# QuantumLab-ZY/HamGNN

Hardware: AMD Instinct MI355X
Metric: edges/sec (equivariant MP forward) (higher is better)
Workload: dtype f32; 1 GPU; sio2_10k: 10002 atoms, 822350 directed edges, irreps set-A (D=877), sh lmax 5, 3 layers, nao_max 19, no SOC, backbone+head forward; parallelism=single GPU

## Files before the change

hamgnn_amd/csrc/tp_is.hip:

```cpp
#include "tp_stage.h"

#ifdef HG_PROF
__device__ unsigned long long hg_prof_is_acc[16];
struct ProfIs { unsigned long long t[12]; unsigned long long last; };
#define IS_PROF_ARG , ProfIs& prof
#define IS_PROF_PASS , prof
#define IS_T(k)                                                      \
    do {                                                             \
        const unsigned long long t_ = __builtin_readcyclecounter();  \
        prof.t[k] += t_ - prof.last;                                 \
        prof.last = t_;                                              \
    } while (0)
#else
#define IS_PROF_ARG
#define IS_PROF_PASS
#define IS_T(k)
#endif
#define IS_MB_CASE(Q) case Q: asm("v_mul_f32_dpp %0, %1, %2 row_newbcast:" #Q " row_mask:0xf bank_mask:0xf" : "=v"(o) : "v"(v), "v"(x)); break;
__device__ __forceinline__ float is_mul_bcast(float v, float x, int q) {
    float o;
    switch (q) {
        IS_MB_CASE(0) IS_MB_CASE(1) IS_MB_CASE(2) IS_MB_CASE(3) IS_MB_CASE(4) IS_MB_CASE(5) IS_MB_CASE(6) IS_MB_CASE(7)
        IS_MB_CASE(8) IS_MB_CASE(9) IS_MB_CASE(10) IS_MB_CASE(11) IS_MB_CASE(12) IS_MB_CASE(13) IS_MB_CASE(14)
        default: asm("v_mul_f32_dpp %0, %1, %2 row_newbcast:15 row_mask:0xf bank_mask:0xf" : "=v"(o) : "v"(v), "v"(x)); break;
    }
    return o;
}
#undef IS_MB_CASE

template <int MM, int RTM, bool SPLIT, bool ODD>
__device__ __forceinline__ void item_is(const IsArgs& A, const float* __restrict__ Wb, const int* __restrict__ it,
                                        float* __restrict__ lds, int64_t erow, int lane, const IsHidden& hbr, int hbr_cls IS_PROF_ARG) {
    constexpr int NCR = 2 * MM + 1;
    constexpr int NC = ODD ? 2 * MM : NCR;
#define IS_COL(c) ((ODD && (c) >= MM) ? (c) + 1 : (c))
#define IS_NK2_OK(rt, r) ((rt) + 1 < RTM || 4 * (rt) + (r) < nk2)
    constexpr int CW = NC > 7 ? (NC + 1) / 2 : NC;
    const int typ = it[0], so0 = it[1], so1 = it[2], in_mulp = it[4], li = it[5], neg = it[7];
    const int ksteps = it[8], mlp = it[10], x4 = it[17], nk2 = it[18];
    const int rto = it[22];
    const int g = lane >> 4, el = lane & 15;
    const int* __restrict__ rtab = reinterpret_cast<const int*>(lds + A.rowtab_off) + it[23];
    float* __restrict__ tbase = lds + (SPLIT ? A.tile_shift : 0) + (el - MM * 16);
    const float* __restrict__ stage = lds + A.stage_off;
    IS_T(0);

    const int nsrc = so1 >= 0 ? 2 : 1;
    const int ngrp = (ksteps + 3) >> 2;
    const f32x4* __restrict__ aw = reinterpret_cast<const f32x4*>(Wb + it[11]) + lane;
    f32x4 av_n[RTM];
    constexpr int NPAIR = RTM * NCR, NJ = (NPAIR + 15) / 16;
    f32x4 cfv[NJ];
    if (typ == 0) {
        const f32x4* __restrict__ cfp = reinterpret_cast<const f32x4*>(Wb + it[13] + NPAIR * 16) + lane;
#pragma unroll
        for (int j = 0; j < NJ; ++j) cfv[j] = cfp[j * 64];
    }
    f32x4 S[RTM];
    if (typ == 0) {
#pragma unroll
        for (int rt = 0; rt < RTM; ++rt) S[rt] = (f32x4){0.f, 0.f, 0.f, 0.f};
        const float* __restrict__ hrow = (mlp ? A.h2[1] : A.h2[0]) + erow * A.hidden + 4 * g;
        const f32x4* __restrict__ w3 = reinterpret_cast<const f32x4*>(Wb + it[12]) + lane;
        const int hgrp = A.hidden >> 4;
        if (mlp == hbr_cls) {
            const f32x4* __restrict__ w3s = w3 + 4 * RTM * 64;
            f32x4 wh[2][RTM], wl[2][RTM], S1[RTM];
#pragma unroll
            for (int t = 0; t < 2; ++t)
#pragma unroll
                for (int rt = 0; rt < RTM; ++rt) {
                    wh[t][rt] = w3s[((t * RTM + rt) * 2) * 64];
                    wl[t][rt] = w3s[((t * RTM + rt) * 2 + 1) * 64];
                }
#pragma unroll
            for (int rt = 0; rt < RTM; ++rt) S1[rt] = (f32x4){0.f, 0.f, 0.f, 0.f};
#ifndef K_S_NOBATCH
            asm volatile("s_waitcnt vmcnt(0)" ::: "memory");
            __builtin_amdgcn_sched_barrier(0);
#endif
#pragma unroll
            for (int t = 0; t < 2; ++t) {
#pragma unroll
                for (int rt = 0; rt < RTM; ++rt) S[rt] = __builtin_amdgcn_mfma_f32_16x16x32_f16(__builtin_bit_cast(f16x8, wh[t][rt]), hbr.hi[t], S[rt], 0, 0, 0);
#pragma unroll
                for (int rt = 0; rt < RTM; ++rt) S1[rt] = __builtin_amdgcn_mfma_f32_16x16x32_f16(__builtin_bit_cast(f16x8, wh[t][rt]), hbr.lo[t], S1[rt], 0, 0, 0);
#pragma unroll
                for (int rt = 0; rt < RTM; ++rt) S1[rt] = __builtin_amdgcn_mfma_f32_16x16x32_f16(__builtin_bit_cast(f16x8, wl[t][rt]), hbr.hi[t], S1[rt], 0, 0, 0);
            }
#ifndef K_S_NOBATCH
            __builtin_amdgcn_sched_barrier(0);
#endif
            const float c0 = A.s_scale, c1 = A.s_scale * (1.f / 2048.f);
#pragma unroll
            for (int rt = 0; rt < RTM; ++rt) S[rt] = S[rt] * c0 + S1[rt] * c1;
        } else
#pragma unroll 1
        for (int G0 = 0; G0 < hgrp; G0 += 4) {
            f32x4 hb[4], wv[4][RTM];
#pragma unroll
            for (int G = 0; G < 4; ++G)
                if (G0 + G < hgrp) {
                    hb[G] = *reinterpret_cast<const f32x4*>(hrow + 16 * (G0 + G));
#pragma unroll
                    for (int rt = 0; rt < RTM; ++rt) wv[G][rt] = w3[((G0 + G) * RTM + rt) * 64];
                }
#pragma unroll
            for (int G = 0; G < 4; ++G)
                if (G0 + G < hgrp) {
#pragma unroll
                    for (int q = 0; q < 4; ++q)
#pragma unroll
                        for (int rt = 0; rt < RTM; ++rt) S[rt] = __builtin_amdgcn_mfma_f32_16x16x4f32(wv[G][rt][q], hb[G][q], S[rt], 0, 0, 0);
                }
        }
    }

    IS_T(1);
#if defined(K_XDL_DUMMY) || defined(K_SMFMA_DUMMY)
#ifdef K_XD_ROLE
    if (typ == 0 && ((blockIdx.x >> 8) & 1)) {
#else
    if (typ == 0) {
#endif
        f32x4 dA[RTM], dB[RTM];
#pragma unroll
        for (int rt = 0; rt < RTM; ++rt) dA[rt] = dB[rt] = (f32x4){0.f, 0.f, 0.f, 0.f};
#ifdef K_XD_DRAIN
// ... 67 lines not shown
#endif
#if defined(K_XD_DRAIN) || defined(K_XD_NOPS)
        __builtin_amdgcn_sched_barrier(0);
        asm volatile("s_nop 15\n s_nop 15\n s_nop 15\n s_nop 15" ::: "memory");
#ifdef K_XD_LONG
#pragma unroll 1
        for (int w_ = 0; w_ < K_XD_LONG; ++w_) asm volatile("s_nop 15\n s_nop 15\n s_nop 15\n s_nop 15" ::: "memory");
#endif
        __builtin_amdgcn_sched_barrier(0);
#endif
#pragma unroll
        for (int rt = 0; rt < RTM; ++rt) asm volatile("" :: "v"(dA[rt]), "v"(dB[rt]));
#if defined(K_XD_DRAIN)
        __builtin_amdgcn_sched_barrier(0);
#endif
    }
#endif
    f32x4 mid[RTM][NC];
#pragma unroll
    for (int rt = 0; rt < RTM; ++rt)
#pragma unroll
        for (int c = 0; c < NC; ++c) mid[rt][c] = (f32x4){0.f, 0.f, 0.f, 0.f};
    const int P1 = in_mulp >> 2;
    const int cdir = neg ? -P1 : P1;
    const int c0p = (li - MM) * P1 + (neg ? (NCR - 1) * P1 : 0);
    const int ntot = nsrc * ngrp;
    const int src_jump = (so1 - so0) - ngrp * 256;
    if (NCR <= 3 && x4) {
        const float* __restrict__ pc[NC];
#pragma unroll
        for (int c = 0; c < NC; ++c) pc[c] = stage + so0 + (c0p + g + IS_COL(c) * cdir) * 64 + el * 4;
#pragma unroll
        for (int rt = 0; rt < RTM; ++rt) av_n[rt] = aw[rt * 64];
#pragma unroll 1
        for (int t = 0; t < ntot; ++t) {
            if (t == ngrp) {
#pragma unroll
                for (int c = 0; c < NC; ++c) pc[c] += src_jump;
            }
            f32x4 av[RTM], bv[NC];
#pragma unroll
            for (int rt = 0; rt < RTM; ++rt) av[rt] = av_n[rt];
            if (t + 1 < ntot) {
#pragma unroll
                for (int rt = 0; rt < RTM; ++rt) av_n[rt] = aw[((t + 1) * RTM + rt) * 64];
            }
#pragma unroll
            for (int c = 0; c < NC; ++c) {
                bv[c] = *reinterpret_cast<const f32x4*>(pc[c]);
                pc[c] += 256;
            }
#pragma unroll
            for (int q = 0; q < 4; ++q)
#pragma unroll
                for (int rt = 0; rt < RTM; ++rt)
#pragma unroll
                    for (int c = 0; c < NC; ++c)
                        mid[rt][c] = __builtin_amdgcn_mfma_f32_16x16x4f32(av[rt][q], bv[c][q], mid[rt][c], 0, 0, 0);
        }
    } else {
        const float* __restrict__ pc[NC];
#pragma unroll
        for (int c = 0; c < NC; ++c) pc[c] = stage + so0 + (c0p + IS_COL(c) * cdir) * 64 + el * 4 + g;
#pragma unroll
        for (int rt = 0; rt < RTM; ++rt) av_n[rt] = aw[rt * 64];
        int nq = ksteps;
#pragma unroll 1
        for (int t = 0; t < ntot; ++t) {
            if (t == ngrp) {
                nq = ksteps;
#pragma unroll
                for (int c = 0; c < NC; ++c) pc[c] += src_jump;
            }
            f32x4 av[RTM];
#pragma unroll
            for (int rt = 0; rt < RTM; ++rt) av[rt] = av_n[rt];
            if (t + 1 < ntot) {
#pragma unroll
                for (int rt = 0; rt < RTM; ++rt) av_n[rt] = aw[((t + 1) * RTM + rt) * 64];
            }
#pragma unroll
            for (int q = 0; q < 4; ++q) {
                if (q < nq) {
                    float b[NC];
#pragma unroll
                    for (int c = 0; c < NC; ++c) b[c] = pc[c][q * 64];
                    __builtin_amdgcn_sched_barrier(0);
#pragma unroll
                    for (int rt = 0; rt < RTM; ++rt)
#pragma unroll
                        for (int c = 0; c < NC; ++c)
                            mid[rt][c] = __builtin_amdgcn_mfma_f32_16x16x4f32(av[rt][q], b[c], mid[rt][c], 0, 0, 0);
                }
            }
            nq -= 4;
#pragma unroll
            for (int c = 0; c < NC; ++c) pc[c] += 256;
        }
    }

    IS_T(2);
    if (typ == 0) {
        const f32x4* __restrict__ a2 = reinterpret_cast<const f32x4*>(Wb + it[14]) + lane;
        const f32x4* __restrict__ cf = reinterpret_cast<const f32x4*>(Wb + it[13]) + g;
        f32x4 a2_n[RTM];
#pragma unroll
        for (int rt = 0; rt < RTM; ++rt) a2_n[rt] = a2[rt * 64];
#pragma unroll
        for (int rt = 0; rt < RTM; ++rt)
#pragma unroll
            for (int c = 0; c < NC; ++c) {
                const int p = rt * NCR + IS_COL(c);
                f32x4 t = mid[rt][c] * S[rt];
#pragma unroll
                for (int r = 0; r < 4; ++r) t[r] = is_mul_bcast(cfv[p >> 4][r], t[r], p & 15);
                mid[rt][c] = t;
            }

        if (CW == NC) {
            float* __restrict__ tnext[4];
            f32x4 acc_n[NC];
#pragma unroll
            for (int r = 0; r < 4; ++r) tnext[r] = tbase + rtab[4 * g + r];
#pragma unroll
            for (int c = 0; c < NC; ++c)
#pragma unroll
                for (int r = 0; r < 4; ++r) acc_n[c][r] = tnext[r][IS_COL(c) * 16];
#pragma unroll 1
            for (int rtp = 0; rtp < rto; ++rtp) {
                f32x4 av[RTM], acc[NC];
                float* __restrict__ trow[4];
#pragma unroll
                for (int rt = 0; rt < RTM; ++rt) av[rt] = a2_n[rt];
// ... 365 lines not shown
#pragma unroll
                        for (int r = 0; r < 4; ++r) tb[rowoff[rtp][r] + (c0 + c) * 16] = acc[c][r];
                    }
            }
        } else {
#pragma unroll 1
            for (int rtp = 0; rtp < RTO; ++rtp) {
                f32x4 avr[RTO], acc[CH];
                int ro[4];
#pragma unroll
                for (int rt = 0; rt < RTO; ++rt) avr[rt] = a2[(rtp * RTO + rt) * 64];
#pragma unroll
                for (int r = 0; r < 4; ++r) ro[r] = rtab[16 * rtp + 4 * g + r];
#pragma unroll
                for (int c = 0; c < CH; ++c) acc[c] = (f32x4){0.f, 0.f, 0.f, 0.f};
#pragma unroll
                for (int rt = 0; rt < RTO; ++rt)
#pragma unroll
                    for (int r = 0; r < 4; ++r)
#pragma unroll
                        for (int c = 0; c < CH; ++c) acc[c] = __builtin_amdgcn_mfma_f32_16x16x4f32(avr[rt][r], md[rt][c][r], acc[c], 0, 0, 0);
#pragma unroll
                for (int c = 0; c < CH; ++c)
                    if (c0 + c < nco) {
#pragma unroll
                        for (int r = 0; r < 4; ++r) tb[ro[r] + (c0 + c) * 16] = acc[c][r];
                    }
            }
        }
    }
}

#define IS_CASE(MMv, RTMv) \
    case (MMv * 8 + RTMv): item_is<MMv, RTMv, SPLIT, false>(A, g_W, it, lds, erow, lane, hbr, hbr_cls IS_PROF_PASS); break;
#define IS_CASE_ODD(MMv, RTMv) \
    case (64 + MMv * 8 + RTMv): item_is<MMv, RTMv, SPLIT, true>(A, g_W, it, lds, erow, lane, hbr, hbr_cls IS_PROF_PASS); break;

#define IS_PART_I32 16

template <bool SPLIT, bool LITE>
__global__ __launch_bounds__(LITE ? 64 * IS_NW_LITE : IS_NT, (LITE ? IS_NW_LITE : IS_NW) / 2) void tp_is_kernel(const IsArgs A0, const int* __restrict__ g_segs, const int* __restrict__ g_blocks,
                                                       const int* __restrict__ g_phases, const int* __restrict__ g_groups,
                                                       const int* __restrict__ g_items, const float* __restrict__ g_W,
                                                       const int* __restrict__ g_parts, const int* __restrict__ g_rowtab) {
    extern __shared__ __attribute__((aligned(16))) float lds[];
    constexpr int NW = LITE ? IS_NW_LITE : IS_NW, NT = 64 * NW;
    const int wave = threadIdx.x >> 6, lane = threadIdx.x & 63;
    const int g = lane >> 4;
    const int64_t e = (int64_t)blockIdx.x * 16 + (lane & 15);
    const bool valid = e < A0.rows;
    const int64_t eslot = valid ? e : A0.rows - 1;
    const int64_t erow = A0.eperm ? A0.eperm[eslot] : eslot;
    const int* __restrict__ PT = g_parts + (SPLIT ? blockIdx.y : 0) * IS_PART_I32;
    IsArgs Asplit;
    if constexpr (SPLIT) {
        Asplit = A0;
        Asplit.trash_off = PT[4];
        Asplit.stage_off = PT[5];
        Asplit.ctr_off = PT[6];
        Asplit.rowtab_off = PT[8];
        Asplit.rowtab_begin = PT[9];
        Asplit.rowtab_len = PT[10];
        Asplit.tile_shift = wave * PT[7];
    }
    const IsArgs& A = SPLIT ? Asplit : A0;
    const int seg0 = SPLIT ? PT[0] : 0, seg1 = SPLIT ? PT[0] + PT[1] : A0.nseg, ph0 = SPLIT ? PT[2] : 0, ph1 = SPLIT ? PT[2] + PT[3] : A0.nphase;
    const int copy_stride = SPLIT ? PT[7] : 0;
    float* __restrict__ stage = lds + A.stage_off;
    int* __restrict__ ctr = reinterpret_cast<int*>(lds + A.ctr_off);
// ... 43 lines not shown
                case 1: stage_block<1, NW>(A, B, stage, erow, wave, lane); break;
                case 2: stage_block<2, NW>(A, B, stage, erow, wave, lane); break;
                case 3: stage_block<3, NW>(A, B, stage, erow, wave, lane); break;
                case 4: stage_block<4, NW>(A, B, stage, erow, wave, lane); break;
                case 5: stage_block<5, NW>(A, B, stage, erow, wave, lane); break;
                case 6: stage_block<6, NW>(A, B, stage, erow, wave, lane); break;
                default: break;
            }
#ifdef HG_PROF
            if (!((A.rot_mask >> B[0]) & 1)) { IS_T(8); } else if (B[4] == 0) { IS_T(9); } else if (B[4] <= 3) { IS_T(10); } else { IS_T(11); }
#endif
        }
        asm volatile("s_waitcnt vmcnt(0)" ::: "memory");
        __syncthreads();
        IS_T(6);
        int gi_dealt = g0 + __builtin_amdgcn_readfirstlane(wave);
        while (true) {
            int gi = 0;
#if defined(IS_DYNAMIC_CLAIM)
            if (false) {
#elif defined(IS_DEAL_ALL)
            if (true) {
#else
            if (SPLIT && copy_stride) {
#endif
                gi = gi_dealt;
                gi_dealt += NW;
            } else {
                if (lane == 0) gi = atomicAdd(ctr, 1);
                gi = __builtin_amdgcn_readfirstlane(gi);
            }
            if (gi >= g1) break;
            const int ib = g_groups[2 * gi], ie = g_groups[2 * gi + 1];
            for (int ii = ib; ii < ie; ++ii) {
                const int* __restrict__ it = g_items + ii * 24;
                if (LITE) {
                    IS_T(0);
                    if (it[0] == 3) {
                        if (it[22] == 1) post_is<1>(A, g_W, it, lds, erow, lane);
                        else if (it[22] == 2) post_is<2>(A, g_W, it, lds, erow, lane);
                        else if (it[22] == 3) post_is<3>(A, g_W, it, lds, erow, lane);
                        else post_is<4>(A, g_W, it, lds, erow, lane);
                    }
                    else if (it[0] == 6) stream_lite(A, g_W, it, lds, lane);
                    else if (it[9] == 1) item_lite<1>(A, g_W, it, lds, lane);
                    else if (it[9] == 2) item_lite<2>(A, g_W, it, lds, lane);
                    else if (it[9] == 3) item_lite<3>(A, g_W, it, lds, lane);
                    else item_lite<4>(A, g_W, it, lds, lane);
                    if (it[0] == 3) { IS_T(3); } else { IS_T(2); }
                    continue;
                }
                switch (it[6] * 8 + it[9] + ((it[0] == 0 && it[7]) ? 64 : 0)) {
                    IS_CASE(0, 1) IS_CASE(0, 2) IS_CASE(0, 3) IS_CASE(0, 4)
                    IS_CASE(1, 1) IS_CASE(1, 2) IS_CASE(1, 3) IS_CASE(1, 4)
                    IS_CASE(2, 1) IS_CASE(2, 2) IS_CASE(2, 3)
                    IS_CASE(3, 1) IS_CASE(3, 2)
                    IS_CASE(4, 1) IS_CASE(4, 2)
                    IS_CASE(5, 1)
                    IS_CASE(6, 1)
                    IS_CASE_ODD(1, 1) IS_CASE_ODD(1, 2) IS_CASE_ODD(1, 3) IS_CASE_ODD(1, 4)
                    IS_CASE_ODD(2, 1) IS_CASE_ODD(2, 2) IS_CASE_ODD(2, 3)
                    IS_CASE_ODD(3, 1) IS_CASE_ODD(3, 2)
                    IS_CASE_ODD(4, 1) IS_CASE_ODD(4, 2)
                    IS_CASE_ODD(5, 1)
                    IS_CASE_ODD(6, 1)
                    default: break;
                }
            }
        }
    }

    if (SPLIT && copy_stride) {
        __syncthreads();
        for (int i = threadIdx.x; i < copy_stride; i += NT) {
            float acc = lds[i];
#pragma unroll
            for (int k = 1; k < NW; ++k) acc += lds[i + k * copy_stride];
            lds[i] = acc;
        }
    }
    IsScan scan;
    scan.last = true, scan.row = 0;
    if (!SPLIT && A0.run_id) scan = is_scan_setup(valid ? A0.run_id[e] : -1 - (int)(lane & 15), lane & 15);
    for (int sg = seg0; sg < seg1; ++sg) {
        const int* __restrict__ S8 = g_segs + sg * 8;
        const int lk = S8[0], mul_k = S8[1], out_off = S8[3], out_mulp = S8[4], tile_off = S8[5], woff = S8[6], flags = S8[7];
        if (sg == seg0 || (flags & SEG_NEWBATCH)) {
            __syncthreads();
            if (flags & SEG_NEWBATCH) {
                int lprev = -1;
                for (int s2 = sg; s2 < seg1; ++s2) {
                    const int* __restrict__ T8 = g_segs + s2 * 8;
                    if (s2 > sg && (T8[7] & SEG_NEWBATCH)) break;
                    const int l2 = T8[0];
                    if (!(T8[7] & SEG_UNROTATE) || l2 == lprev) continue;
                    lprev = l2;
                    const int nn = (2 * l2 + 1) * (2 * l2 + 1);
                    const float* __restrict__ D = A.wig + erow * A.nW + is_pick_wig_off(A, l2);
                    const int nj = (nn + 3) >> 2;
// ... 53 lines not shown

extern "C" int hg_tp_is(const float* const* src, const int64_t* src_stride, int nsrc, const float* h2_node, const float* h2_edge,
                        int hidden, const float* wig, int nW, const int32_t* wig_off, const float* weights, const int32_t* seg_table,
                        const int32_t* block_table, const int32_t* phase_table, const int32_t* group_table,
                        const int32_t* item_table, const int32_t* part_table, const int32_t* part_table_host, int nparts,
                        const int32_t* row_table, int lds_bytes,
                        const int64_t* const* src_idx, int rot_mask, const int64_t* edge_perm, const int32_t* run_id, float* out, int64_t out_stride,
                        int64_t rows, void* stream) {
    HgDeviceGuard dev_guard(stream);
    if (rows <= 0) return 0;
    if (nsrc < 1 || nsrc > 4) return hg_fail(-2, "hg_tp_is: nsrc must be 1..4");
    if (hidden & 15) return hg_fail(-2, "hg_tp_is: (padded) hidden width must be a multiple of 16");
    if (lds_bytes <= 0 || lds_bytes > 160 * 1024) return hg_fail(-2, "hg_tp_is: bad LDS size");
    if (!part_table || !part_table_host || nparts < 1 || nparts > 64) return hg_fail(-2, "hg_tp_is: 1..64 parts");
    IsArgs A;
    for (int i = 0; i < 4; ++i) {
        A.src[i] = i < nsrc ? src[i] : src[0];
        A.sstride[i] = i < nsrc ? src_stride[i] : src_stride[0];
    }
    A.h2[0] = h2_node;
    A.h2[1] = h2_edge;
    A.hidden = hidden;
    A.wig = wig;
    A.nW = nW;
    for (int i = 0; i < 8; ++i) A.wig_off[i] = wig_off ? wig_off[i] : 0;
    A.out = out;
    A.ostride = out_stride;
    A.rows = rows;
    A.tile_shift = 0;
    const int32_t* p0 = part_table_host;
    A.nseg = p0[1], A.nphase = p0[3], A.trash_off = p0[4], A.stage_off = p0[5], A.ctr_off = p0[6];
    A.rowtab_off = p0[8], A.rowtab_begin = p0[9], A.rowtab_len = p0[10];
    A.s_split = p0[12] == 1 && hidden == 64;
    A.s_scale = ldexpf(1.f, -(p0[13] + IS_SPLIT_H_EXP));
    if (!row_table) return hg_fail(-2, "hg_tp_is: no row table");
    for (int p = 0; p < nparts; ++p) {
        const int32_t* q = part_table_host + p * IS_PART_I32;
        if (q[6] < q[5] || q[5] < q[8] + q[10] || q[8] < q[4] || lds_bytes < 4 * (q[6] + 1) || (q[7] && (part_table_host[11] ? IS_NW_LITE : IS_NW) * q[7] > q[8]))
            return hg_fail(-2, "hg_tp_is: bad LDS layout");
    }
    for (int i = 0; i < 4; ++i) A.idx[i] = (src_idx && i < nsrc) ? src_idx[i] : nullptr;
    A.rot_mask = rot_mask;
    A.eperm = edge_perm;
    A.run_id = run_id;
    if (run_id && nparts != 1) return hg_fail(-2, "hg_tp_is: the fused scatter needs a single-part launch");
    if (rot_mask && !wig) return hg_fail(-2, "hg_tp_is: rotated sources need the Wigner rows");
    static unsigned char lds_attr_done[4][HG_MAX_DEVICES];
    if (int rc = hg_lds_attr_once(lds_attr_done[0], dev_guard.dev, (const void*)tp_is_kernel<false, false>, 160 * 1024)) return rc;
    if (int rc = hg_lds_attr_once(lds_attr_done[1], dev_guard.dev, (const void*)tp_is_kernel<true, false>, 160 * 1024)) return rc;
    if (int rc = hg_lds_attr_once(lds_attr_done[2], dev_guard.dev, (const void*)tp_is_kernel<false, true>, 160 * 1024)) return rc;
    if (int rc = hg_lds_attr_once(lds_attr_done[3], dev_guard.dev, (const void*)tp_is_kernel<true, true>, 160 * 1024)) return rc;
    const unsigned grid = (unsigned)((rows + 15) / 16);
    const bool lite = p0[11] != 0;
#define IS_LAUNCH(SPLITv, LITEv, GRID) \
    hipLaunchKernelGGL((tp_is_kernel<SPLITv, LITEv>), GRID, dim3(LITEv ? 64 * IS_NW_LITE : IS_NT), lds_bytes, (hipStream_t)stream, A, seg_table, block_table, phase_table, \
                       group_table, item_table, weights, part_table, row_table)
    if (nparts == 1) {
        if (lite) IS_LAUNCH(false, true, dim3(grid));
        else IS_LAUNCH(false, false, dim3(grid));
    } else {
        if (lite) IS_LAUNCH(true, true, dim3(grid, (unsigned)nparts));
        else IS_LAUNCH(true, false, dim3(grid, (unsigned)nparts));
    }
#undef IS_LAUNCH
    return hg_check_launch("hg_tp_is");
}
// ... 1 lines not shown
```

hamgnn_amd/csrc/tp_stage.h:

```cpp
#pragma once
#include <hip/hip_runtime.h>
#include <stdint.h>
#include "hg_common.h"

typedef float f32x4 __attribute__((ext_vector_type(4)));
typedef _Float16 f16x8 __attribute__((ext_vector_type(8)));
struct IsHidden { f16x8 hi[2], lo[2]; };
#define IS_SPLIT_H_EXP 6
#define IS_SPLIT_H_SCALE 64.f

#ifndef IS_NW
#define IS_NW 4
#endif
#define IS_NT (64 * IS_NW)
#ifndef IS_NW_LITE
#define IS_NW_LITE 8
#endif

struct IsArgs {
    const float* src[4];
    int64_t sstride[4];
    const float* h2[2];
    int hidden;
    const float* wig;
    int nW;
    int wig_off[8];
    float* out;
    int64_t ostride;
    int64_t rows;
    int nseg;
    int nphase;
    int trash_off;
    int stage_off;
    int ctr_off;
    int rowtab_off;
    int rowtab_begin;
    int rowtab_len;
    int tile_shift;
    int s_split;
    float s_scale;
    const int64_t* idx[4];
    int rot_mask;
    const int64_t* eperm;
    const int32_t* run_id;
};

struct IsScan {
    float m[4];
    bool last;
    int row;
};
template <int CTRL>
__device__ __forceinline__ int is_dpp_i(int v) { return __builtin_amdgcn_update_dpp(0, v, CTRL, 0xf, 0xf, true); }
template <int CTRL>
__device__ __forceinline__ float is_dpp_f(float v) { return __builtin_bit_cast(float, __builtin_amdgcn_update_dpp(0, __builtin_bit_cast(int, v), CTRL, 0xf, 0xf, true)); }
__device__ __forceinline__ IsScan is_scan_setup(int rid, int el) {
    IsScan sc;
    sc.row = rid;
    const int prev = is_dpp_i<0x111>(rid), next = is_dpp_i<0x101>(rid);
    int f = (el == 0 || prev != rid) ? 1 : 0;
    sc.last = el == 15 || next != rid;
    sc.m[0] = f ? 0.f : 1.f;
    int f1 = f | (el < 1 ? 1 : is_dpp_i<0x111>(f));
    sc.m[1] = f1 ? 0.f : 1.f;
    int f2 = f1 | (el < 2 ? 1 : is_dpp_i<0x112>(f1));
    sc.m[2] = f2 ? 0.f : 1.f;
    int f4 = f2 | (el < 4 ? 1 : is_dpp_i<0x114>(f2));
    sc.m[3] = f4 ? 0.f : 1.f;
    return sc;
}
__device__ __forceinline__ float is_seg_scan(float x, const IsScan& sc) {
    x = fmaf(sc.m[0], is_dpp_f<0x111>(x), x);
    x = fmaf(sc.m[1], is_dpp_f<0x112>(x), x);
// ... 227 lines not shown
```

hamgnn_amd/ops.py:

```python
from __future__ import annotations

import ctypes as C
import math
import os
from typing import List, Optional, Sequence

import numpy as np
import torch

from . import plan as P
from ._lib import check, f32, i32, i64, lib, ptr


def _stream():
    return C.c_void_p(torch.cuda.current_stream().cuda_stream)


def _on_tensor_device(fn):
    import functools

    @functools.wraps(fn)
    def wrapped(*args, **kwargs):
        for a in args:
            t = a if torch.is_tensor(a) else (a[0] if isinstance(a, (list, tuple)) and a and torch.is_tensor(a[0]) else None)
# ... 4 lines not shown
                break
        return fn(*args, **kwargs)
    return wrapped


def _dev(arr: np.ndarray, device, dtype=None):
    t = torch.from_numpy(np.ascontiguousarray(arr))
    if dtype is not None:
        t = t.to(dtype)
    return t.to(device)


def require_fp32(module, data=None):
    why = None
    if torch.get_default_dtype() == torch.float64:
        why = "torch.get_default_dtype() is float64"
    elif module is not None and next((p.dtype for p in module.parameters()), None) == torch.float64:
        why = "the model's parameters are float64"
    elif data is not None:
        pos = data["pos"] if isinstance(data, dict) else getattr(data, "pos", None)
        if torch.is_tensor(pos) and pos.dtype == torch.float64:
            why = "data.pos is float64"
    if why:
        raise NotImplementedError(f"precision: 64 is not built ({why}): the MI355X path computes in fp32 and does not down-cast silently "
                                  "(reference: hamgnn/main.py:469-474)")


def _require_gpu(t: torch.Tensor):
    if not t.is_cuda:
        raise RuntimeError("hamgnn_amd: the MI355X hot path needs CUDA(ROCm) tensors; there is no CPU fallback")


S_SPLIT_OFF = os.environ.get("HG_S_SPLIT", "1") == "0"
W3_SPLIT_PENDING: list = []
REPLAY_SPLIT = False
REPLAY_SPLIT_TILES = int(os.environ.get("HG_REPLAY_SPLIT_TILES", "1024"))


_BUILD_CONFIG_OK = False


def check_build_config():
    global _BUILD_CONFIG_OK
    if _BUILD_CONFIG_OK:
        return
    L = lib()
    want = {0: ("HG_IS_WAVES", P.IS_WAVES), 1: ("HG_LITE_WAVES", P.IS_WAVES_LITE), 2: ("HG_LITE_SRING", P.LITE_SRING)}
    for what, (name, val) in want.items():
        got = int(L.hg_build_config(what))
        if got != int(val):
            raise RuntimeError(f"{name}={val} does not match the loaded library (compiled with {got}): rebuild the variant or unset the variable")
    _BUILD_CONFIG_OK = True


def w3_split_refill(w: torch.Tensor, se, so, dh, dl, scale: float, lo_scale: float) -> torch.Tensor:
    _require_gpu(w)
    assert w.dtype == torch.float32 and w.is_contiguous() and all(t.dtype == torch.int64 and t.is_contiguous() for t in (se, so, dh, dl))
    mx = torch.empty(1, device=w.device, dtype=torch.float32)
    check(lib().hg_w3_split_refill(ptr(w), ptr(se), ptr(so), ptr(dh), ptr(dl), i64(se.numel()), C.c_float(scale), C.c_float(lo_scale), ptr(mx), _stream()), "hg_w3_split_refill")
    return mx[0]


def check_w3_split():
    if not W3_SPLIT_PENDING:
        return
    pend = list(W3_SPLIT_PENDING)
# ... 23 lines not shown
            raise ValueError("a program with merged items runs on the input-stationary kernel only")
        self.fixed_parts = None
        if schedule in ("is", "auto", "is_parts"):
            try:
                self.sched = self.is_tables(1)[0]
            except NotImplementedError:
                if schedule == "is":
                    raise
                if schedule == "is_parts":
                    self.sched = self.is_tables("lds")[0]
                    self.fixed_parts = "lds"

    def weights_changed(self):
        self.refresh_w3_split()
        self._is_weights.clear()
        self._is_tables = {k: v for k, v in self._is_tables.items() if v[0].extra_weights is None}

    def refresh_w3_split(self):
        regs = getattr(self.prog, "w3_regions", None)
        if not regs:
            return
        if getattr(self, "_w3_idx", None) is None:
            se, so, dh, dl = [], [], [], []
            for off, rtm in regs:
                n = 4 * rtm * 256
                src, dst = P.w3_split_index(rtm)
                se.append(off + src[:, 0]); so.append(off + src[:, 1]); dh.append(off + n + dst[0]); dl.append(off + n + dst[1])
            self._w3_idx = tuple(_dev(np.concatenate(a).astype(np.int64), self._device) for a in (se, so, dh, dl))
        se, so, dh, dl = self._w3_idx
        sc_, lo_ = float(2.0 ** int(getattr(self.prog, "w3_exp", 0))), float(2.0 ** P.SPLIT_LO_EXP)
        W3_SPLIT_PENDING.append((self, w3_split_refill(self.weights, se, so, dh, dl, sc_, lo_)))

    def part_table_host(self, sc) -> np.ndarray:
        if (getattr(self, "_w3_split_off", False) or S_SPLIT_OFF) and int(sc.part_table[0][12]):
            pt = sc.part_table.copy()
            pt[:, 12] = 0
            return pt
        return sc.part_table

    def is_tables(self, parts):
        if parts not in self._is_tables:
            sc = P.is_schedule(self.prog, parts)
            self._is_tables[parts] = (sc, tuple(_dev(t, self._device) for t in (sc.seg_table, sc.block_table, sc.phase_table, sc.group_table,
                                                                                  sc.item_table, sc.part_table, sc.rowtab)))
            if sc.extra_weights is not None:
                self._is_weights[parts] = torch.cat([self.weights, _dev(sc.extra_weights, self._device, torch.float32)])
        return self._is_tables[parts]

    def is_weights(self, parts) -> torch.Tensor:
        return self._is_weights.get(parts, self.weights)

    def is_parts_for(self, rows: int) -> int:
        if self.fixed_parts is not None:
            return self.fixed_parts
        forced = os.environ.get("HG_IS_PARTS")
        if forced:
            return max(1, int(forced))
        tiles = (rows + 15) // 16
        nseg = int(self.prog.seg_table.shape[0])
        mode = os.environ.get("HG_REPLAY_SPLIT", "2d4" if REPLAY_SPLIT else "0")
        if mode.startswith("2d") and tiles * nseg * int(mode[2:] or 3) <= REPLAY_SPLIT_TILES and not int(self.sched.part_table[0][11]):
            return ("2d", nseg, int(mode[2:] or 3))
        if tiles * nseg <= 512:
            return nseg
        if tiles <= 300 and nseg >= 8:
            return 8
        return 1


# ... 597 lines not shown
```

hamgnn_amd/plan/schedule_is.py:

```python
from __future__ import annotations

import os
from dataclasses import dataclass, field
from typing import Dict, List, Optional, Tuple

import numpy as np

from ._blas import single_thread_blas
from .layout import ITEM_I32, IT_LIN, IT_LINC, IT_LINM, IT_POST, IT_STREAM, IT_TP, LITE_SRING, SEG_I32, SEG_UNROTATE, ceil_div

IS_WAVES = int(os.environ.get("HG_IS_WAVES", "4"))
IS_WAVES_LITE = int(os.environ.get("HG_LITE_WAVES", "8"))
IS_BLOCK_I32 = 8
IS_PHASE_I32 = 8
IS_LDS_BYTES = 80 * 1024
IS_ITEM_I32 = 24


@dataclass
class IsSchedule:
    seg_table: np.ndarray
    block_table: np.ndarray
    phase_table: np.ndarray
    group_table: np.ndarray
    item_table: np.ndarray
    part_table: np.ndarray
    rowtab: np.ndarray
    lds_floats: int
    balance: float
    part_cost: List[int]
    phase_cls: List[int] = field(default_factory=list)
    extra_weights: Optional[np.ndarray] = None
    atomic_out: bool = False

    @property
    def trash_off(self):
        return int(self.part_table[0][4])

    @property
    def stage_off(self):
        return int(self.part_table[0][5])

    @property
    def ctr_off(self):
        return int(self.part_table[0][6])

    @property
    def stage_floats(self):
# ... 45 lines not shown
            if bins[b] + sz <= cap:
                bins[b] += sz
                break
        else:
            b = len(bins)
            bins.append(sz)
        for m in units[key]:
            owner[m] = b
    return owner


@single_thread_blas
def is_schedule(prog: "Program", parts=1, separate_mlp: Optional[bool] = None) -> IsSchedule:
    phase_chunks = 1
    if isinstance(parts, tuple):
        assert parts[0] == "2d"
        parts, phase_chunks = int(parts[1]), max(1, int(parts[2]))
    if separate_mlp is None:
        plain = is_schedule(prog, parts if phase_chunks == 1 else ("2d", parts, phase_chunks), separate_mlp=False)
        if (parts != 1 and os.environ.get("HG_SEP_PARTS") != "1") or prog.hidden != 64:
            return plain
        try:
            sep = is_schedule(prog, parts, separate_mlp=True)
        except NotImplementedError:
            return plain
        return sep if sum(sep.part_cost) <= 1.01 * sum(plain.part_cost) else plain
    if separate_mlp and np.isin(prog.item_table[:, 0], (IT_LINC, IT_LINM, IT_POST)).any():
        raise NotImplementedError("lite_mode programs have no per-generator phases")
    hp4 = prog.hidden_pad // 4
    nseg = prog.seg_table.shape[0]
    lite_flag = int(np.isin(prog.item_table[:, 0], (IT_LINC, IT_LINM, IT_POST)).any())
    s_split = int(bool(getattr(prog, "w3_regions", None)) and getattr(prog, "w3_split_ok", True))
    s_exp = int(getattr(prog, "w3_exp", 0))
    if lite_flag and np.isin(prog.item_table[:, 0], (IT_TP, IT_LIN)).any():
        raise NotImplementedError("input-stationary schedule: a program mixes lite_mode items with tensor-product / Linear items")
    key_of = [prog.seg_key.get(sg, sg) for sg in range(nseg)]
    seg_cost = np.zeros(nseg)
    for rec in prog.item_table:
        seg_cost[key_of[int(rec[19])]] += _item_cost(rec, prog.seg_table, hp4, prog.vsegs)
    owner = np.zeros(nseg, dtype=np.int64)
    nkeys = len(set(key_of))
    if parts == "lds":
        owner = np.asarray(lds_partition(prog), dtype=np.int64)
        parts = int(owner.max()) + 1
    else:
        parts = max(1, min(int(parts), nkeys))
    if parts > 1 and not owner.any():
        load, held = [0.0] * parts, [0] * parts
        for sg in np.argsort(-seg_cost, kind="stable"):
            if key_of[sg] != sg:
                continue
            r = min(range(parts), key=lambda q: (load[q], held[q], q))
            load[r] += seg_cost[sg]
            held[r] += 1
            for m in range(nseg):
                if key_of[m] == sg:
                    owner[m] = r
    runs = dict(base=int(prog.weights.size), w=[]) if (prog.item_table[:, 0] == IT_LINM).any() else None
    segs_all, btab, ptab, gtab, items_all, parttab, part_cost, rowtab_all = [], [], [], [], [], [], [], []
    phase_cls_all: List[int] = []
    lds_floats, worst_balance = 0, 1.0
    atomic_any = False
    for part in range(parts):
        members = [sg for sg in range(nseg) if owner[sg] == part]
        sub = _is_schedule_part(prog, members, hp4, seg_base=len(segs_all), block_base=len(btab), group_base=len(gtab), item_base=len(items_all),
                                split=parts > 1, separate_mlp=separate_mlp, runs=runs, waves=IS_WAVES_LITE if lite_flag else IS_WAVES)
        nph_ = len(sub["ptab"])
        K_ = min(phase_chunks, nph_) if (phase_chunks > 1 and parts > 1 and not lite_flag) else 1
        if K_ > 1:
            bins_: List[List[int]] = [[] for _ in range(K_)]
            ld_ = [0] * K_
            for ph in sorted(range(nph_), key=lambda p_: -sub["phase_crit"][p_]):
                b_ = min(range(K_), key=lambda q: (ld_[q], q))
                bins_[b_].append(ph)
                ld_[b_] += sub["phase_crit"][ph] + 150
            order_ = [ph for b_ in bins_ for ph in b_]
            sub["ptab"] = [sub["ptab"][ph] for ph in order_]
            sub["phase_cls"] = [sub["phase_cls"][ph] for ph in order_]
            sub["segs"][:, 7] |= SEG_ATOMIC
            o_ = 0
            for b_ in bins_:
                parttab.append([len(segs_all), len(sub["segs"]), len(ptab) + o_, len(b_), sub["trash_off"], sub["stage_off"], sub["ctr_off"],
                                sub["copy_stride"], sub["rowtab_off"], len(rowtab_all), len(sub["rowtab"]), lite_flag, s_split, s_exp, 0, 0])
                o_ += len(b_)
            atomic_any = True
        else:
            parttab.append([len(segs_all), len(sub["segs"]), len(ptab), len(sub["ptab"]), sub["trash_off"], sub["stage_off"], sub["ctr_off"],
                            sub["copy_stride"], sub["rowtab_off"], len(rowtab_all), len(sub["rowtab"]), lite_flag, s_split, s_exp, 0, 0])
        rowtab_all += sub["rowtab"]
        phase_cls_all += sub["phase_cls"]
        segs_all += list(sub["segs"])
        btab += sub["btab"]
        ptab += sub["ptab"]
        gtab += sub["gtab"]
        items_all += list(sub["items"])
        lds_floats = max(lds_floats, sub["ctr_off"] + 4)
        worst_balance = min(worst_balance, sub["balance"])
        part_cost.append(sub["crit"])
    items = np.asarray(items_all, np.int32).reshape(-1, IS_ITEM_I32)
    return IsSchedule(np.asarray(segs_all, np.int32).reshape(-1, SEG_I32), np.asarray(btab, np.int32).reshape(-1, IS_BLOCK_I32),
                      np.asarray(ptab, np.int32).reshape(-1, IS_PHASE_I32), np.asarray(gtab, np.int32).reshape(-1, 2), items,
                      np.ascontiguousarray(np.asarray(parttab, np.int32).reshape(-1, IS_PART_I32)), np.asarray(rowtab_all, np.int32),
                      lds_floats, worst_balance, part_cost, phase_cls_all,
                      extra_weights=(np.concatenate(runs["w"]) if runs is not None and runs["w"] else None), atomic_out=atomic_any)


def _lite_column_steps(prog: "Program", items, lk: int, rtm: int, pairing: bool):
    Wt = prog.weights

    def item_steps(r, m):
        so0, so1, in_mulp, li, mm, neg, ksteps, a1, colstride = int(r[1]), int(r[2]), int(r[4]), int(r[5]), int(r[6]), int(r[7]), int(r[8]), int(r[11]), int(r[13])
        if abs(m) > mm:
            return None
        c = m + mm
        nsrc, ngrp, P1 = (2 if so1 >= 0 else 1), ceil_div(ksteps, 4), in_mulp // 4
        cdir = -P1 if neg else P1
        c0p = (li - mm) * P1 + ((2 * mm) * P1 if neg else 0)
        st = []
        for si in range(nsrc):
            for G in range(ngrp):
                base = (so1 if si else so0) + (c0p + c * cdir + 4 * G) * 64
# ... 253 lines not shown
        else:
            batches.append([l])
    woff, batch_of = {}, {}
    for bi, bt in enumerate(batches):
        o = 0
        for l in bt:
            woff[l], batch_of[l] = o, bi
            o += need[l]
    order = sorted(range(len(segs)), key=lambda i: (batch_of.get(int(segs[i][0]), -1) if int(segs[i][7]) & SEG_UNROTATE else -1))
    remap = {members[old]: seg_base + new for new, old in enumerate(order)}
    segs2 = segs[order].copy()
    prev = None
    for sg in segs2:
        if int(sg[7]) & SEG_UNROTATE:
            l = int(sg[0])
            sg[6] = woff[l]
            if batch_of[l] != prev:
                sg[7] |= SEG_NEWBATCH
                prev = batch_of[l]
    items = np.asarray(items, np.int32).reshape(-1, ITEM_I32)
    wide = np.zeros((items.shape[0], IS_ITEM_I32), np.int32)
    wide[:, :ITEM_I32] = items
    for n in range(items.shape[0]):
        g_abs = remap[int(items[n, 19])]
        sg = segs2[g_abs - seg_base]
        wide[n, 19] = g_abs
        wide[n, 20], wide[n, 21], wide[n, 22], wide[n, 23] = sg[0], sg[1], sg[2], rt_base[order[g_abs - seg_base]]
        v = int(items[n, 16]) - 1 if int(items[n, 0]) == IT_TP else -1
        if v >= 0:
            wide[n, 22], wide[n, 23] = _item_rto(items[n], prog.seg_table, prog.vsegs), vt_base[v]
    ctr_off = stage_off + stage_floats
    return dict(segs=segs2.astype(np.int32), btab=btab, ptab=ptab, gtab=gtab, items=wide, trash_off=trash_off, stage_off=stage_off, remap=remap,
                phase_crit=phase_crit, phase_touch=phase_touch, phase_cls=phase_cls, rowtab=rowtab, rowtab_off=rowtab_off, ctr_off=ctr_off, copy_stride=copy_stride, balance=tot / (waves * crit) if crit else 1.0, crit=crit)
```

Baseline: 4.060 million edges/s.

## Compute next item's split-f16 hidden GEMM ahead during current item's main loop

Adds a look-ahead in the input-stationary tensor-product kernel. Before the main MFMA loop of each item, it issues the next item's W3 split-weight loads, and after the loop it computes that item's radial-scale S vector (with at most 2 row tiles) and carries it in registers to the next item. The goal is to hide the global-load latency of the W3 weights behind the current item's compute. In exchange it uses more VGPRs, which may lower occupancy, and adds per-item branching; it is gated by a part-table flag and an env var.

Measured after the change: 3.895 million edges/s. -4.0%, worse.

```diff
diff --git a/hamgnn_amd/csrc/tp_is.hip b/hamgnn_amd/csrc/tp_is.hip
--- a/hamgnn_amd/csrc/tp_is.hip
+++ b/hamgnn_amd/csrc/tp_is.hip
@@ -28,9 +28,53 @@
 }
 #undef IS_MB_CASE
 
+template <int NRT, int LD>
+__device__ __forceinline__ void is_scale_split(const f32x4 (&wh)[2][LD], const f32x4 (&wl)[2][LD], const IsHidden& hbr, float s_scale, f32x4* __restrict__ S) {
+    f32x4 S1[NRT];
+#pragma unroll
+    for (int rt = 0; rt < NRT; ++rt) S[rt] = S1[rt] = (f32x4){0.f, 0.f, 0.f, 0.f};
+#ifndef K_S_NOBATCH
+    asm volatile("s_waitcnt vmcnt(0)" ::: "memory");
+    __builtin_amdgcn_sched_barrier(0);
+#endif
+#pragma unroll
+    for (int t = 0; t < 2; ++t) {
+#pragma unroll
+        for (int rt = 0; rt < NRT; ++rt) S[rt] = __builtin_amdgcn_mfma_f32_16x16x32_f16(__builtin_bit_cast(f16x8, wh[t][rt]), hbr.hi[t], S[rt], 0, 0, 0);
+#pragma unroll
+        for (int rt = 0; rt < NRT; ++rt) S1[rt] = __builtin_amdgcn_mfma_f32_16x16x32_f16(__builtin_bit_cast(f16x8, wh[t][rt]), hbr.lo[t], S1[rt], 0, 0, 0);
+#pragma unroll
+        for (int rt = 0; rt < NRT; ++rt) S1[rt] = __builtin_amdgcn_mfma_f32_16x16x32_f16(__builtin_bit_cast(f16x8, wl[t][rt]), hbr.hi[t], S1[rt], 0, 0, 0);
+    }
+#ifndef K_S_NOBATCH
+    __builtin_amdgcn_sched_barrier(0);
+#endif
+    const float c0 = s_scale, c1 = s_scale * (1.f / 2048.f);
+#pragma unroll
+    for (int rt = 0; rt < NRT; ++rt) S[rt] = S[rt] * c0 + S1[rt] * c1;
+}
+__device__ __forceinline__ void is_ahead_request(const float* __restrict__ Wb, int w3_off, int nrt, int lane, f32x4 (&wh)[2][IS_AHEAD_RT], f32x4 (&wl)[2][IS_AHEAD_RT]) {
+    const f32x4* __restrict__ w3s = reinterpret_cast<const f32x4*>(Wb + w3_off) + lane + 4 * nrt * 64;
+    if (nrt >= 1) {
+#pragma unroll
+        for (int t = 0; t < 2; ++t) {
+            wh[t][0] = w3s[((t * nrt) * 2) * 64];
+            wl[t][0] = w3s[((t * nrt) * 2 + 1) * 64];
+        }
+        if (nrt >= 2) {
+#pragma unroll
+            for (int t = 0; t < 2; ++t) {
+                wh[t][1] = w3s[((t * 2 + 1) * 2) * 64];
+                wl[t][1] = w3s[((t * 2 + 1) * 2 + 1) * 64];
+            }
+        }
+    }
+}
+
 template <int MM, int RTM, bool SPLIT, bool ODD>
 __device__ __forceinline__ void item_is(const IsArgs& A, const float* __restrict__ Wb, const int* __restrict__ it,
-                                        float* __restrict__ lds, int64_t erow, int lane, const IsHidden& hbr, int hbr_cls IS_PROF_ARG) {
+                                        float* __restrict__ lds, int64_t erow, int lane, const IsHidden& hbr, int hbr_cls, IsAhead& ah,
+                                        const int* __restrict__ nit IS_PROF_ARG) {
     constexpr int NCR = 2 * MM + 1;
     constexpr int NC = ODD ? 2 * MM : NCR;
 #define IS_COL(c) ((ODD && (c) >= MM) ? (c) + 1 : (c))
@@ -43,6 +87,13 @@
     const int* __restrict__ rtab = reinterpret_cast<const int*>(lds + A.rowtab_off) + it[23];
     float* __restrict__ tbase = lds + (SPLIT ? A.tile_shift : 0) + (el - MM * 16);
     const float* __restrict__ stage = lds + A.stage_off;
+    const int* __restrict__ nx = nit ? nit : it;
+    const int n_typ = nx[0], n_rtm = nx[9], n_mlp = nx[10], n_w3 = nx[12];
+    const int nrt = (nit && n_typ == 0 && n_mlp == hbr_cls && n_rtm <= IS_AHEAD_RT) ? n_rtm : 0;
+    f32x4 nwh[2][IS_AHEAD_RT], nwl[2][IS_AHEAD_RT];
+    bool own_s = true;
+    if constexpr (RTM <= IS_AHEAD_RT) own_s = !ah.valid;
+    ah.valid = 0;
     IS_T(0);
 
     const int nsrc = so1 >= 0 ? 2 : 1;
@@ -57,7 +108,12 @@
         for (int j = 0; j < NJ; ++j) cfv[j] = cfp[j * 64];
     }
     f32x4 S[RTM];
-    if (typ == 0) {
+    if (typ == 0 && !own_s) {
+        if constexpr (RTM <= IS_AHEAD_RT) {
+#pragma unroll
+            for (int rt = 0; rt < RTM; ++rt) S[rt] = ah.S[rt];
+        }
+    } else if (typ == 0) {
 #pragma unroll
         for (int rt = 0; rt < RTM; ++rt) S[rt] = (f32x4){0.f, 0.f, 0.f, 0.f};
         const float* __restrict__ hrow = (mlp ? A.h2[1] : A.h2[0]) + erow * A.hidden + 4 * g;
@@ -65,7 +121,7 @@
         const int hgrp = A.hidden >> 4;
         if (mlp == hbr_cls) {
             const f32x4* __restrict__ w3s = w3 + 4 * RTM * 64;
-            f32x4 wh[2][RTM], wl[2][RTM], S1[RTM];
+            f32x4 wh[2][RTM], wl[2][RTM];
 #pragma unroll
             for (int t = 0; t < 2; ++t)
 #pragma unroll
@@ -73,27 +129,7 @@
                     wh[t][rt] = w3s[((t * RTM + rt) * 2) * 64];
                     wl[t][rt] = w3s[((t * RTM + rt) * 2 + 1) * 64];
                 }
-#pragma unroll
-            for (int rt = 0; rt < RTM; ++rt) S1[rt] = (f32x4){0.f, 0.f, 0.f, 0.f};
-#ifndef K_S_NOBATCH
-            asm volatile("s_waitcnt vmcnt(0)" ::: "memory");
-            __builtin_amdgcn_sched_barrier(0);
-#endif
-#pragma unroll
-            for (int t = 0; t < 2; ++t) {
-#pragma unroll
-                for (int rt = 0; rt < RTM; ++rt) S[rt] = __builtin_amdgcn_mfma_f32_16x16x32_f16(__builtin_bit_cast(f16x8, wh[t][rt]), hbr.hi[t], S[rt], 0, 0, 0);
-#pragma unroll
-                for (int rt = 0; rt < RTM; ++rt) S1[rt] = __builtin_amdgcn_mfma_f32_16x16x32_f16(__builtin_bit_cast(f16x8, wh[t][rt]), hbr.lo[t], S1[rt], 0, 0, 0);
-#pragma unroll
-                for (int rt = 0; rt < RTM; ++rt) S1[rt] = __builtin_amdgcn_mfma_f32_16x16x32_f16(__builtin_bit_cast(f16x8, wl[t][rt]), hbr.hi[t], S1[rt], 0, 0, 0);
-            }
-#ifndef K_S_NOBATCH
-            __builtin_amdgcn_sched_barrier(0);
-#endif
-            const float c0 = A.s_scale, c1 = A.s_scale * (1.f / 2048.f);
-#pragma unroll
-            for (int rt = 0; rt < RTM; ++rt) S[rt] = S[rt] * c0 + S1[rt] * c1;
+            is_scale_split<RTM, RTM>(wh, wl, hbr, A.s_scale, S);
         } else
 #pragma unroll 1
         for (int G0 = 0; G0 < hgrp; G0 += 4) {
@@ -227,6 +263,7 @@
         for (int c = 0; c < NC; ++c) pc[c] = stage + so0 + (c0p + g + IS_COL(c) * cdir) * 64 + el * 4;
 #pragma unroll
         for (int rt = 0; rt < RTM; ++rt) av_n[rt] = aw[rt * 64];
+        is_ahead_request(Wb, n_w3, nrt, lane, nwh, nwl);
 #pragma unroll 1
         for (int t = 0; t < ntot; ++t) {
             if (t == ngrp) {
@@ -259,6 +296,7 @@
         for (int c = 0; c < NC; ++c) pc[c] = stage + so0 + (c0p + IS_COL(c) * cdir) * 64 + el * 4 + g;
 #pragma unroll
         for (int rt = 0; rt < RTM; ++rt) av_n[rt] = aw[rt * 64];
+        is_ahead_request(Wb, n_w3, nrt, lane, nwh, nwl);
         int nq = ksteps;
 #pragma unroll 1
         for (int t = 0; t < ntot; ++t) {
@@ -294,6 +332,13 @@
         }
     }
 
+    if (nrt == 1) {
+        is_scale_split<1, IS_AHEAD_RT>(nwh, nwl, hbr, A.s_scale, ah.S);
+        ah.valid = 1;
+    } else if (nrt == 2) {
+        is_scale_split<2, IS_AHEAD_RT>(nwh, nwl, hbr, A.s_scale, ah.S);
+        ah.valid = 1;
+    }
     IS_T(2);
     if (typ == 0) {
         const f32x4* __restrict__ a2 = reinterpret_cast<const f32x4*>(Wb + it[14]) + lane;
@@ -725,9 +770,9 @@
 }
 
 #define IS_CASE(MMv, RTMv) \
-    case (MMv * 8 + RTMv): item_is<MMv, RTMv, SPLIT, false>(A, g_W, it, lds, erow, lane, hbr, hbr_cls IS_PROF_PASS); break;
+    case (MMv * 8 + RTMv): item_is<MMv, RTMv, SPLIT, false>(A, g_W, it, lds, erow, lane, hbr, hbr_cls, ah, nit IS_PROF_PASS); break;
 #define IS_CASE_ODD(MMv, RTMv) \
-    case (64 + MMv * 8 + RTMv): item_is<MMv, RTMv, SPLIT, true>(A, g_W, it, lds, erow, lane, hbr, hbr_cls IS_PROF_PASS); break;
+    case (64 + MMv * 8 + RTMv): item_is<MMv, RTMv, SPLIT, true>(A, g_W, it, lds, erow, lane, hbr, hbr_cls, ah, nit IS_PROF_PASS); break;
 
 #define IS_PART_I32 16
 
@@ -837,8 +882,11 @@
             }
             if (gi >= g1) break;
             const int ib = g_groups[2 * gi], ie = g_groups[2 * gi + 1];
+            IsAhead ah;
+            ah.valid = 0;
             for (int ii = ib; ii < ie; ++ii) {
                 const int* __restrict__ it = g_items + ii * 24;
+                const int* __restrict__ nit = (!LITE && A.s_ahead && ii + 1 < ie) ? it + 24 : nullptr;
                 if (LITE) {
                     IS_T(0);
                     if (it[0] == 3) {
@@ -869,7 +917,7 @@
                     IS_CASE_ODD(4, 1) IS_CASE_ODD(4, 2)
                     IS_CASE_ODD(5, 1)
                     IS_CASE_ODD(6, 1)
-                    default: break;
+                    default: ah.valid = 0; break;
                 }
             }
         }
@@ -989,6 +1037,7 @@
     A.nseg = p0[1], A.nphase = p0[3], A.trash_off = p0[4], A.stage_off = p0[5], A.ctr_off = p0[6];
     A.rowtab_off = p0[8], A.rowtab_begin = p0[9], A.rowtab_len = p0[10];
     A.s_split = p0[12] == 1 && hidden == 64;
+    A.s_ahead = p0[14] == 1;
     A.s_scale = ldexpf(1.f, -(p0[13] + IS_SPLIT_H_EXP));
     if (!row_table) return hg_fail(-2, "hg_tp_is: no row table");
     for (int p = 0; p < nparts; ++p) {
diff --git a/hamgnn_amd/csrc/tp_stage.h b/hamgnn_amd/csrc/tp_stage.h
--- a/hamgnn_amd/csrc/tp_stage.h
+++ b/hamgnn_amd/csrc/tp_stage.h
@@ -8,6 +8,8 @@
 struct IsHidden { f16x8 hi[2], lo[2]; };
 #define IS_SPLIT_H_EXP 6
 #define IS_SPLIT_H_SCALE 64.f
+#define IS_AHEAD_RT 2
+struct IsAhead { f32x4 S[IS_AHEAD_RT]; int valid; };
 
 #ifndef IS_NW
 #define IS_NW 4
@@ -39,6 +41,7 @@
     int tile_shift;
     int s_split;
     float s_scale;
+    int s_ahead;
     const int64_t* idx[4];
     int rot_mask;
     const int64_t* eperm;
diff --git a/hamgnn_amd/ops.py b/hamgnn_amd/ops.py
--- a/hamgnn_amd/ops.py
+++ b/hamgnn_amd/ops.py
@@ -60,6 +60,7 @@
 
 
 S_SPLIT_OFF = os.environ.get("HG_S_SPLIT", "1") == "0"
+S_AHEAD_OFF = os.environ.get("HG_S_AHEAD", "1") == "0"
 W3_SPLIT_PENDING: list = []
 REPLAY_SPLIT = False
 REPLAY_SPLIT_TILES = int(os.environ.get("HG_REPLAY_SPLIT_TILES", "1024"))
@@ -149,9 +150,14 @@
         W3_SPLIT_PENDING.append((self, w3_split_refill(self.weights, se, so, dh, dl, sc_, lo_)))
 
     def part_table_host(self, sc) -> np.ndarray:
-        if (getattr(self, "_w3_split_off", False) or S_SPLIT_OFF) and int(sc.part_table[0][12]):
+        split_off = (getattr(self, "_w3_split_off", False) or S_SPLIT_OFF) and int(sc.part_table[0][12])
+        ahead_off = S_AHEAD_OFF and int(sc.part_table[0][14])
+        if split_off or ahead_off:
             pt = sc.part_table.copy()
-            pt[:, 12] = 0
+            if split_off:
+                pt[:, 12] = 0
+            if ahead_off:
+                pt[:, 14] = 0
             return pt
         return sc.part_table
 
diff --git a/hamgnn_amd/plan/schedule_is.py b/hamgnn_amd/plan/schedule_is.py
--- a/hamgnn_amd/plan/schedule_is.py
+++ b/hamgnn_amd/plan/schedule_is.py
@@ -14,6 +14,7 @@
 IS_BLOCK_I32 = 8
 IS_PHASE_I32 = 8
 IS_LDS_BYTES = 80 * 1024
+AHEAD_RT = 2
 IS_ITEM_I32 = 24
 
 
@@ -125,6 +126,7 @@
     lite_flag = int(np.isin(prog.item_table[:, 0], (IT_LINC, IT_LINM, IT_POST)).any())
     s_split = int(bool(getattr(prog, "w3_regions", None)) and getattr(prog, "w3_split_ok", True))
     s_exp = int(getattr(prog, "w3_exp", 0))
+    s_ahead = int(bool(s_split) and not lite_flag)
     if lite_flag and np.isin(prog.item_table[:, 0], (IT_TP, IT_LIN)).any():
         raise NotImplementedError("input-stationary schedule: a program mixes lite_mode items with tensor-product / Linear items")
     key_of = [prog.seg_key.get(sg, sg) for sg in range(nseg)]
@@ -174,12 +176,12 @@
             o_ = 0
             for b_ in bins_:
                 parttab.append([len(segs_all), len(sub["segs"]), len(ptab) + o_, len(b_), sub["trash_off"], sub["stage_off"], sub["ctr_off"],
-                                sub["copy_stride"], sub["rowtab_off"], len(rowtab_all), len(sub["rowtab"]), lite_flag, s_split, s_exp, 0, 0])
+                                sub["copy_stride"], sub["rowtab_off"], len(rowtab_all), len(sub["rowtab"]), lite_flag, s_split, s_exp, s_ahead, 0])
                 o_ += len(b_)
             atomic_any = True
         else:
             parttab.append([len(segs_all), len(sub["segs"]), len(ptab), len(sub["ptab"]), sub["trash_off"], sub["stage_off"], sub["ctr_off"],
-                            sub["copy_stride"], sub["rowtab_off"], len(rowtab_all), len(sub["rowtab"]), lite_flag, s_split, s_exp, 0, 0])
+                            sub["copy_stride"], sub["rowtab_off"], len(rowtab_all), len(sub["rowtab"]), lite_flag, s_split, s_exp, s_ahead, 0])
         rowtab_all += sub["rowtab"]
         phase_cls_all += sub["phase_cls"]
         segs_all += list(sub["segs"])
@@ -499,3 +501,27 @@
     ctr_off = stage_off + stage_floats
     return dict(segs=segs2.astype(np.int32), btab=btab, ptab=ptab, gtab=gtab, items=wide, trash_off=trash_off, stage_off=stage_off, remap=remap,
                 phase_crit=phase_crit, phase_touch=phase_touch, phase_cls=phase_cls, rowtab=rowtab, rowtab_off=rowtab_off, ctr_off=ctr_off, copy_stride=copy_stride, balance=tot / (waves * crit) if crit else 1.0, crit=crit)
+
+
+def ahead_coverage(sc: IsSchedule) -> Dict[str, int]:
+    out = dict(ahead_1=0, ahead_2=0, too_tall=0, other_mlp=0, linear=0, first=0, single_groups=0, items=int(sc.item_table.shape[0]), groups=0)
+    for part in sc.part_table:
+        for ph in range(int(part[2]), int(part[2]) + int(part[3])):
+            g0, g1, cls = (int(v) for v in sc.phase_table[ph][2:5])
+            for gi in range(g0, g1):
+                ib, ie = (int(v) for v in sc.group_table[gi])
+                if ie <= ib:
+                    continue
+                out["groups"] += 1
+                out["first"] += 1
+                out["single_groups"] += int(ie - ib == 1)
+                for rec in sc.item_table[ib + 1:ie]:
+                    if int(rec[0]) != IT_TP:
+                        out["linear"] += 1
+                    elif cls < 0 or int(rec[10]) != cls:
+                        out["other_mlp"] += 1
+                    elif int(rec[9]) > AHEAD_RT:
+                        out["too_tall"] += 1
+                    else:
+                        out["ahead_%d" % int(rec[9])] += 1
+    return out
```
